# zju3dv/OnePose_Plus_Plus

Hardware: AMD Instinct MI355X
Metric: query images/sec (2D-3D match fwd) at 512x512 img x 5k pts (higher is better)
Workload: dtype f32 (operands as exact bf16 triples, f32 accumulate)

## Files before the change

onepose_plus_plus_amd/csrc/gemm_mfma.hip:

```cpp
#include <stdlib.h>

#include <mutex>
#include <type_traits>

#include <vector>

#include "opp_internal.h"

typedef float f32x16 __attribute__((ext_vector_type(16)));
typedef _Float16 f16x8 __attribute__((ext_vector_type(8)));
typedef __bf16 bf16x8 __attribute__((ext_vector_type(8)));
typedef __bf16 bf16x2 __attribute__((ext_vector_type(2)));
typedef float f32x2 __attribute__((ext_vector_type(2)));

namespace {

constexpr int lds_stride(int prec) { return prec == OPP_PREC_BF16X3 ? 52 : 36; }

__device__ __forceinline__ void opp_split4_b3(const float4 v, uint2& hi, uint2& mid, uint2& lo) {
  auto lvl = [](float a, float b, float& ra, float& rb) -> unsigned {
    const f32x2 t = {a, b};
    const unsigned p = __builtin_bit_cast(unsigned, __builtin_convertvector(t, bf16x2));
    ra = a - __uint_as_float(p << 16);
    rb = b - __uint_as_float(p & 0xffff0000u);
// ... 9 lines not shown
}
__device__ __forceinline__ void opp_store_split4(void* base, size_t row_bytes_off, int col, const float4 v) {
  uint2 hi, mid, lo;
  opp_split4_b3(v, hi, mid, lo);
  char* p = static_cast<char*>(base) + row_bytes_off + (col >> 3) * 48 + (col & 7) * 2;
  *reinterpret_cast<uint2*>(p) = hi;
  *reinterpret_cast<uint2*>(p + 16) = mid;
  *reinterpret_cast<uint2*>(p + 32) = lo;
}

template <int BM, int BN, int WAVES_M, int WAVES_N, bool CONV, int ABL, int DEPTH, int PREC, bool ASP>
__device__ __forceinline__ void opp_gemm_body(const OppGemm& g) {
  constexpr bool H2 = PREC == OPP_PREC_FP16X2;
  constexpr bool H3 = PREC == OPP_PREC_BF16X3;
  constexpr int kLdsStride = lds_stride(PREC);
  constexpr int NT = WAVES_M * WAVES_N * 64;
  constexpr int TM = BM / WAVES_M / 32;
  constexpr int NT32 = BN / 32;
  constexpr int TN = (NT32 + WAVES_N - 1) / WAVES_N;
  constexpr bool kRagged = (NT32 % WAVES_N) != 0;
  static_assert(!ASP || (CONV && PREC == OPP_PREC_BF16X3 && (ABL == 0 || ABL >= 200)), "pre-split activations: bf16x3 convolutions only");
  constexpr int kAblMask = ABL >= 200 ? ABL - 200 : 0;
  constexpr bool kNoGload = ABL == 91 || (kAblMask & 1), kNoLdsSt = ABL == 92 || (kAblMask & 2), kNoBar = ABL == 93 || (kAblMask & 4),
                 kNoFrag = ABL == 94 || (kAblMask & 8);
  constexpr int A_LD = ASP ? (BM * 12 + NT - 1) / NT : BM * 8 / NT;
  constexpr bool kAFrac = ASP && (BM * 12) % NT != 0;
  constexpr int kBRowsLoad = (H3 && BN == 224) ? 208 : BN;
  constexpr int B_LD = H3 ? (kBRowsLoad * 12 + NT - 1) / NT : BN * 8 / NT;
  constexpr bool kBFrac = H3 && (kBRowsLoad * 12) % NT != 0;
  constexpr bool kRing = H3 && kRagged && !CONV;
  constexpr bool kM16 = H3 && CONV;
  constexpr int NB16 = kM16 ? kBRowsLoad / 16 : 1;
  constexpr int NBW = kM16 ? (NB16 + WAVES_N - 1) / WAVES_N : 1;
  constexpr int MB = 2 * TM;
  static_assert(!kM16 || (kBRowsLoad % 16 == 0 && (!kRagged || WAVES_N == 2)), "16 x 16 tile shape");
  static_assert(BM % (WAVES_M * 32) == 0 && BN % 32 == 0, "tile shape");
  static_assert((BM * 8) % NT == 0 && (H3 ? (BN * 12) % NT == 0 || BN == 192 || BN == 224 : (BN * 8) % NT == 0), "load split");
  static_assert(!ASP || !((H3 && ((BN + 31) / 32 % WAVES_N) != 0)), "pre-split activations are not built for the ring tile");

  unsigned long long ts0 = 0, ts1 = 0, ts2 = 0;
  if (ABL == 9 || ABL > 90) ts0 = __builtin_readcyclecounter();
  extern __shared__ __attribute__((aligned(16))) float smem[];
  float* As = smem;
  float* Bs = smem + 2 * BM * kLdsStride;

  const int tid = threadIdx.x;
  const int lane = tid & 63;
  const int wave = tid >> 6;
  const int wm = __builtin_amdgcn_readfirstlane((H3 && kRagged) ? wave % WAVES_M : wave / WAVES_N);
  const int wn = __builtin_amdgcn_readfirstlane((H3 && kRagged) ? wave / WAVES_M : wave % WAVES_N);
  bool tile_ok[TN];
#pragma unroll
  for (int j = 0; j < TN; ++j) tile_ok[j] = kRagged ? (wn * TN + j < NT32) : true;
  const int half = lane >> 5;
  const int l31 = lane & 31;

  const int tiles_n = (g.n_store + BN - 1) / BN;
  int tile_lin = blockIdx.x;
  if (g.xcd_swizzle & 1) {
    const int nb = gridDim.x, q = nb >> 3, r = nb & 7;
    const int xcd = blockIdx.x & 7, idx = blockIdx.x >> 3;
    tile_lin = (xcd < r ? xcd * (q + 1) : r * (q + 1) + (xcd - r) * q) + idx;
  }
  const int tile_m = tile_lin / tiles_n;
  const int tile_n = tile_lin - tile_m * tiles_n;
  const int m0 = tile_m * BM;
  const int n0 = tile_n * BN;

// ... 9 lines not shown
#pragma unroll
  for (int i = 0; i < A_LD; ++i) {
    const int au = tid + i * NT;
    const int arow = ASP ? au / 12 : lrow + i * (NT / 8);
    const int apiece = ASP ? au - arow * 12 : 0;
    if constexpr (ASP) a_lds[i] = piece_off(arow, apiece);
    const int r = m0 + arow;
    if (CONV) {
      const int ox = r % g.Wout;
      const int t = r / g.Wout;
      const int oy = t % g.Hout;
      const int b = t / g.Hout;
      const int iy0 = oy * g.stride - g.pad;
      const int ix0 = ox * g.stride - g.pad;
      if constexpr (ASP) a_base0[i] = (unsigned)(((b * g.Hin + iy0) * g.Win + ix0) * g.Cin) * 6u + (unsigned)apiece * 16u;
      else a_base0[i] = (unsigned)(((b * g.Hin + iy0) * g.Win + ix0) * g.Cin + kq * 4) * 4u;
      a_base1[i] = 0;
      unsigned m = 0;
#pragma unroll
      for (int ky = 0; ky < 3; ++ky)
#pragma unroll
        for (int kx = 0; kx < 3; ++kx) {
          const bool ok = ky < g.ksize && kx < g.ksize && (unsigned)(iy0 + ky) < (unsigned)g.Hin &&
                          (unsigned)(ix0 + kx) < (unsigned)g.Win;
          m |= (ok ? 1u : 0u) << (ky * g.ksize + kx);
        }
      a_mask[i] = (r < g.M && (!kAFrac || au < BM * 12)) ? ~m : 0xffffffffu;
    } else {
      a_base0[i] = r < g.M ? (unsigned)(r * g.lda0 + kq * 4) * 4u : kOob;
      a_base1[i] = r < g.M ? (unsigned)(r * g.lda1 + kq * 4) * 4u : kOob;
      a_mask[i] = 0;
    }
  }
  constexpr bool kRingB = H3 && (NT32 % WAVES_N) != 0;
  unsigned b_base[kRingB ? 1 : B_LD];
  int b_lds[kRingB ? 1 : B_LD];
  auto ring_b = [&](int i, unsigned& base, int& lds) {
    int t = tid;
    asm volatile("" : "+v"(t));
    const int u = t + i * NT;
    const int row = u / 12, c = u - row * 12;
    const int n = n0 + row;
    base = (n < g.N && u < kBRowsLoad * 12) ? (unsigned)(n * g.ldw + c * 4) * 4u : kOob;
    lds = row * kLdsStride + c * 4;
  };
#pragma unroll
  for (int i = 0; i < (kRingB ? 0 : B_LD); ++i) {
    if (H3) {
      const int u = tid + i * NT;
      const int row = u / 12, c = u - row * 12;
      const int n = n0 + row;
      if constexpr (kBFrac) b_base[i] = (n < g.N && u < kBRowsLoad * 12) ? (unsigned)(n * g.ldw + c * 4) * 4u : kOob;
      else b_base[i] = n < g.N ? (unsigned)(n * g.ldw + c * 4) * 4u : kOob;
      b_lds[i] = piece_off(row, c);
    } else {
      const int n = n0 + lrow + i * (NT / 8);
      b_base[i] = n < g.N ? (unsigned)(n * g.ldw + kq * 4) * 4u : kOob;
      b_lds[i] = (lrow + i * (NT / 8)) * kLdsStride + kq * 4;
    }
  }

  typedef unsigned int u32x4 __attribute__((ext_vector_type(4)));
  auto bload = [](const __amdgpu_buffer_rsrc_t r, unsigned off) -> float4 {
    const u32x4 v = __builtin_amdgcn_raw_buffer_load_b128(r, (int)off, 0, 0);
    return make_float4(__uint_as_float(v.x), __uint_as_float(v.y), __uint_as_float(v.z), __uint_as_float(v.w));
  };

// ... 471 lines not shown
    mfma_ring(0, 2, 5, 2 * TM * TNW, tnw_c, pre);
    __builtin_amdgcn_sched_barrier(0);
    read_frags_n(B0, 4, fa[2], fb[2], tnw_c);
    __builtin_amdgcn_sched_barrier(0);
    mfma_ring(0, 5, 6, 5 * TM * TNW, tnw_c, pre);
#pragma unroll
    for (int i = kSlotsR0 / kStrideR0; i < A_LD; ++i) load_item(i, ga[P], gb[0]);
    __builtin_amdgcn_sched_barrier(0);
    mfma_ring(1, 0, 3, 0, tnw_c, [&](int n) {
      if (n % kStrideR1 == 0 && n / kStrideR1 < kItems) {
        store_item(n / kStrideR1, B1, ga[PN], gb[0]);
        __builtin_amdgcn_sched_barrier(0);
      }
    });
#pragma unroll
    for (int i = kSlotsR1 / kStrideR1; i < kItems; ++i) store_item(i, B1, ga[PN], gb[0]);
    __builtin_amdgcn_sched_barrier(0);
    __syncthreads();
    read_frags_n(B1, 0, fa[0], fb[0], tnw_c);
    read_frags_n(B1, 2, fa[3], fb[3], tnw_c);
    __builtin_amdgcn_sched_barrier(0);
    mfma_ring(1, 3, 5, 0, tnw_c, pre_b);
    __builtin_amdgcn_sched_barrier(0);
    read_frags_n(B1, 1, fa[2], fb[2], tnw_c);
    __builtin_amdgcn_sched_barrier(0);
    mfma_ring(1, 5, 6, 2 * TM * TNW, tnw_c, pre_b);
#pragma unroll
    for (int i = kSlotsR1 / kStrideRB; i < B_LD; ++i) load_item(A_LD + i, ga[P], gb[0]);
    __builtin_amdgcn_sched_barrier(0);
  };


  typedef float f32x4 __attribute__((ext_vector_type(4)));
  constexpr int NBH0 = (NBW + 1) / 2;
  f32x4 acc4[kM16 ? MB : 1][kM16 ? NBW : 1];
  float4 fa4[3][kM16 ? MB : 1], fb4[3][kM16 ? NBW : 1];
  if constexpr (kM16) {
#pragma unroll
    for (int i = 0; i < MB; ++i)
#pragma unroll
      for (int j = 0; j < NBW; ++j) acc4[i][j] = f32x4{0.f, 0.f, 0.f, 0.f};
  }
  const int f16off = (lane & 15) * kLdsStride + (((lane >> 4) ^ kswz(lane & 15)) * 3) * 4;
  const int a_frag16 = wm * TM * 32 * kLdsStride + f16off;
  const int b_frag16 = wn * NBW * 16 * kLdsStride + f16off;
  auto read_a16 = [&](int buf, auto h_c) {
    constexpr int H = decltype(h_c)::value;
    const float* as = As + buf * BM * kLdsStride + a_frag16;
#pragma unroll
    for (int i = H * TM; i < H * TM + TM; ++i)
#pragma unroll
      for (int p = 0; p < 3; ++p) fa4[p][i] = *reinterpret_cast<const float4*>(as + i * 16 * kLdsStride + p * 4);
  };
  auto read_b16 = [&](int buf, auto v_c, auto nbw_c) {
    constexpr int V = decltype(v_c)::value, NBL = decltype(nbw_c)::value;
    constexpr int j0 = V ? NBH0 : 0, j1 = V ? NBL : (NBH0 < NBL ? NBH0 : NBL);
    const float* bs = Bs + buf * BN * kLdsStride + b_frag16;
#pragma unroll
    for (int j = j0; j < j1; ++j)
#pragma unroll
      for (int p = 0; p < 3; ++p) fb4[p][j] = *reinterpret_cast<const float4*>(bs + j * 16 * kLdsStride + p * 4);
  };
  auto quad16 = [&](auto h_c, auto v_c, auto nbw_c, auto&& between) {
    constexpr int H = decltype(h_c)::value, V = decltype(v_c)::value, NBL = decltype(nbw_c)::value;
    constexpr int j0 = V ? NBH0 : 0, j1 = V ? NBL : (NBH0 < NBL ? NBH0 : NBL);
    constexpr int PA[6] = {2, 0, 1, 1, 0, 0};
    constexpr int PB[6] = {0, 2, 1, 0, 1, 0};
    int n = 0;
#pragma unroll
    for (int pr = 0; pr < 6; ++pr)
#pragma unroll
      for (int i = H * TM; i < H * TM + TM; ++i)
#pragma unroll
        for (int j = j0; j < j1; ++j) {
          acc4[i][j] = __builtin_amdgcn_mfma_f32_16x16x32_bf16(as_b8(fa4[PA[pr]][i]), as_b8(fb4[PB[pr]][j]), acc4[i][j], 0, 0, 0);
          between(n);
          ++n;
        }
  };
  auto chunk_m16 = [&](auto set, int lb, auto nbw_c) {
    constexpr int P = decltype(set)::value;
    constexpr int NBL = decltype(nbw_c)::value;
    constexpr int O = P & 1;
    constexpr int kSl0 = 6 * TM * (O ? NBL - NBH0 : (NBH0 < NBL ? NBH0 : NBL));
    constexpr int kSl1 = 6 * TM * (O ? (NBH0 < NBL ? NBH0 : NBL) : NBL - NBH0);
    constexpr int kSt0 = kSl0 / kItems > 0 ? kSl0 / kItems : 1;
    constexpr int kSt1 = kSl1 / kItems > 0 ? kSl1 / kItems : 1;
    using I0 = std::integral_constant<int, 0>;
    using I1 = std::integral_constant<int, 1>;
    const int B0 = lb, B1 = lb ^ 1;
    advance();
    if (!kNoFrag) {
      if constexpr (O == 0) read_b16(B0, I1{}, nbw_c);
      else read_b16(B0, I0{}, nbw_c);
      read_a16(B0, I1{});
    }
    __builtin_amdgcn_sched_barrier(0);
    auto hand = [&](int n) {
      if (n % kSt0 == 0 && n / kSt0 < kItems) {
        if (!kNoLdsSt) store_item(n / kSt0, B1, ga[0], gb[0]);
        __builtin_amdgcn_sched_barrier(0);
      }
    };
    auto pre = [&](int n) {
      if (n % kSt1 == 0 && n / kSt1 < kItems) {
        if (!kNoGload) load_item(n / kSt1, ga[0], gb[0]);
        __builtin_amdgcn_sched_barrier(0);
      }
    };
    if constexpr (O == 0) quad16(I0{}, I0{}, nbw_c, hand);
    else quad16(I0{}, I1{}, nbw_c, hand);
#pragma unroll
    for (int i = kSl0 / kSt0; i < kItems; ++i)
      if (!kNoLdsSt) store_item(i, B1, ga[0], gb[0]);
    __builtin_amdgcn_sched_barrier(0);
    if constexpr (O == 0) quad16(I0{}, I1{}, nbw_c, pre);
    else quad16(I0{}, I0{}, nbw_c, pre);
#pragma unroll
    for (int i = kSl1 / kSt1; i < kItems; ++i)
      if (!kNoGload) load_item(i, ga[0], gb[0]);
    __builtin_amdgcn_sched_barrier(0);
    if (!kNoBar) __syncthreads();
    if (!kNoFrag) read_a16(B1, I0{});
    __builtin_amdgcn_sched_barrier(0);
    if constexpr (O == 0) quad16(I1{}, I1{}, nbw_c, nothing);
    else quad16(I1{}, I0{}, nbw_c, nothing);
    __builtin_amdgcn_sched_barrier(0);
    if (!kNoFrag) {
      if constexpr (O == 0) read_b16(B1, I1{}, nbw_c);
      else read_b16(B1, I0{}, nbw_c);
    }
    __builtin_amdgcn_sched_barrier(0);
    if constexpr (O == 0) quad16(I1{}, I0{}, nbw_c, nothing);
    else quad16(I1{}, I1{}, nbw_c, nothing);
    __builtin_amdgcn_sched_barrier(0);
  };
  if constexpr (kM16) {
    if (!kNoFrag) {
      read_a16(0, std::integral_constant<int, 0>{});
      read_b16(0, std::integral_constant<int, 0>{}, std::integral_constant<int, NBW>{});
    }
  }

  if (ABL == 9 || ABL > 90) ts1 = __builtin_readcyclecounter();
  if (NT == 512 && (g.xcd_swizzle & 2) && __builtin_amdgcn_readfirstlane(tid) >= 256) __builtin_amdgcn_s_setprio(1);
  if constexpr (kRing) {
    constexpr int kFull = TN, kShort = NT32 - (WAVES_N - 1) * TN;
    static_assert(DEPTH == 2 && kShort >= 1 && kShort <= TN, "ring tile");
    if (wn != WAVES_N - 1) {
      for (int c = 0; c < nk; c += 2) {
        chunk_ring(std::integral_constant<int, 0>{}, c & 1, std::integral_constant<int, kFull>{});
        chunk_ring(std::integral_constant<int, 1>{}, (c + 1) & 1, std::integral_constant<int, kFull>{});
      }
    } else {
      for (int c = 0; c < nk; c += 2) {
        chunk_ring(std::integral_constant<int, 0>{}, c & 1, std::integral_constant<int, kShort>{});
        chunk_ring(std::integral_constant<int, 1>{}, (c + 1) & 1, std::integral_constant<int, kShort>{});
      }
    }
  }
  if constexpr (kM16) {
    static_assert(DEPTH == 2, "16 x 16 loop: the two quadrant orders alternate over a chunk pair");
    constexpr int kShort16 = NB16 - (WAVES_N - 1) * NBW;
    if (!kRagged || wn != WAVES_N - 1) {
      for (int c = 0; c < nk; c += 2) {
        chunk_m16(std::integral_constant<int, 0>{}, c & 1, std::integral_constant<int, NBW>{});
        chunk_m16(std::integral_constant<int, 1>{}, (c + 1) & 1, std::integral_constant<int, NBW>{});
      }
    } else {
      for (int c = 0; c < nk; c += 2) {
        chunk_m16(std::integral_constant<int, 0>{}, c & 1, std::integral_constant<int, kShort16>{});
        chunk_m16(std::integral_constant<int, 1>{}, (c + 1) & 1, std::integral_constant<int, kShort16>{});
      }
    }
  }
  for (int c = 0; c < ((kRing || kM16) ? 0 : nk); c += DEPTH) {
    if constexpr (kRing || kM16) {
    } else if constexpr (H3) {
      chunk_h3(std::integral_constant<int, 0>{}, c & 1);
      if (DEPTH > 1) chunk_h3(std::integral_constant<int, 1 % DEPTH>{}, (c + 1) & 1);
      if (DEPTH > 2) chunk_h3(std::integral_constant<int, 2 % DEPTH>{}, (c + 2) & 1);
      if (DEPTH > 3) chunk_h3(std::integral_constant<int, 3 % DEPTH>{}, (c + 3) & 1);
    } else if constexpr (H2) {
      chunk_h2(std::integral_constant<int, 0>{}, c & 1);
      if (DEPTH > 1) chunk_h2(std::integral_constant<int, 1 % DEPTH>{}, (c + 1) & 1);
      if (DEPTH > 2) chunk_h2(std::integral_constant<int, 2 % DEPTH>{}, (c + 2) & 1);
      if (DEPTH > 3) chunk_h2(std::integral_constant<int, 3 % DEPTH>{}, (c + 3) & 1);
    } else {
      chunk(std::integral_constant<int, 0>{}, c & 1);
      if (DEPTH > 1) chunk(std::integral_constant<int, 1 % DEPTH>{}, (c + 1) & 1);
      if (DEPTH > 2) chunk(std::integral_constant<int, 2 % DEPTH>{}, (c + 2) & 1);
      if (DEPTH > 3) chunk(std::integral_constant<int, 3 % DEPTH>{}, (c + 3) & 1);
    }
  }
  if (ABL == 9 || ABL > 90) ts2 = __builtin_readcyclecounter();
  if (ABL == 5) {
#pragma unroll
    for (int i = 0; i < A_LD; ++i) asm volatile("" ::"v"(da[i].x), "v"(da[i].w));
#pragma unroll
    for (int i = 0; i < B_LD; ++i) asm volatile("" ::"v"(db[i].x), "v"(db[i].w));
  }

  constexpr int kJPmax = TN < 4 ? TN : 4;
  constexpr int kOperandFloats = 2 * (BM + BN) * kLdsStride;
  constexpr int JP = (BM * (WAVES_N * kJPmax * 32 + 4) <= kOperandFloats) ? kJPmax
                     : (BM * (WAVES_N * 2 * 32 + 4) <= kOperandFloats && kJPmax >= 2) ? 2 : 1;
  constexpr int NPASS = kM16 ? 1 : (TN + JP - 1) / JP;
  constexpr int WP = kM16 ? BN : WAVES_N * JP * 32;
  constexpr int CS = WP + 4;
  static_assert((size_t)BM * CS * 4 <= (size_t)2 * (BM + BN) * kLdsStride * 4, "C tile must fit the operand LDS");
  float* Cs = smem;
  const bool scale_on = (g.out_mul != 1.f) || (g.out_div != 1.f);
  const bool vec_ok = g.vec_epilogue != 0;
  const float h2_inv = (H2 && g.h2_inv != nullptr) ? *g.h2_inv : 1.f;
  if constexpr (kM16) {
    if (scale_on) {
#pragma unroll
      for (int i = 0; i < MB; ++i)
#pragma unroll
        for (int j = 0; j < NBW; ++j)
#pragma unroll
          for (int r = 0; r < 4; ++r) acc4[i][j][r] = (acc4[i][j][r] * g.out_mul) / g.out_div;
    }
  } else if (H2 || scale_on) {
#pragma unroll
    for (int i = 0; i < TM; ++i)
#pragma unroll
      for (int j = 0; j < TN; ++j)
#pragma unroll
        for (int r = 0; r < 16; ++r) {
          const float cv0 = H2 ? acc[i][j][r] * h2_inv : acc[i][j][r];
          acc[i][j][r] = scale_on ? (cv0 * g.out_mul) / g.out_div : cv0;
        }
  }
  if (!kM16 && g.col_mask != nullptr) {
#pragma unroll
    for (int j = 0; j < TN; ++j) {
      const int col = n0 + wn * TN * 32 + j * 32 + l31;
      const float add = (col < g.n_store && g.col_mask[col] == 0.f) ? -1e9f : 0.f;
#pragma unroll
      for (int i = 0; i < TM; ++i)
#pragma unroll
        for (int r = 0; r < 16; ++r) acc[i][j][r] += add;
    }
  }
  if constexpr (H2) {
    if (g.nonfinite != nullptr) {
      bool bad = false;
#pragma unroll
      for (int i = 0; i < TM; ++i)
#pragma unroll
        for (int j = 0; j < TN; ++j)
#pragma unroll
          for (int r = 0; r < 16; ++r) bad |= !(fabsf(acc[i][j][r]) <= 3.4028235e38f);
      if (__builtin_amdgcn_ballot_w64(bad) != 0ull && lane == 0) atomicOr(g.nonfinite, 1);
    }
  }
#pragma unroll
  for (int ps = 0; ps < NPASS; ++ps) {
    __syncthreads();
    if constexpr (kM16) {
#pragma unroll
      for (int i = 0; i < MB; ++i)
#pragma unroll
        for (int j = 0; j < NBW; ++j)
#pragma unroll
          for (int r = 0; r < 4; ++r)
            Cs[(wm * TM * 32 + i * 16 + (lane >> 4) * 4 + r) * CS + wn * NBW * 16 + j * 16 + (lane & 15)] = acc4[i][j][r];
    } else
#pragma unroll
    for (int i = 0; i < TM; ++i)
#pragma unroll
      for (int jj = 0; jj < JP; ++jj) {
        const int j = ps * JP + jj;
        if (j < TN && tile_ok[j]) {
#pragma unroll
          for (int r = 0; r < 16; ++r) {
            const int lr = wm * TM * 32 + i * 32 + (r & 3) + 8 * (r >> 2) + 4 * half;
            Cs[lr * CS + wn * JP * 32 + jj * 32 + l31] = acc[i][j][r];
          }
        }
      }
    __syncthreads();
    if constexpr (!kM16 && NPASS == 1 && !kRagged && (NT % BM) == 0 && kOperandFloats - BM * CS >= 2 * (NT / BM) * BM + 2 * WAVES_M * WP) {
      if (g.stat_rowmax != nullptr) {
        constexpr int kParts = NT / BM;
        constexpr int kQ = WP / 4 / kParts;
        float* sc_r = Cs + BM * CS;
        float* sc_c = sc_r + 2 * kParts * BM;
        const int ncols = min(WP, g.n_store - n0);
        const int nrows = min(BM, g.M - m0);
        {
          const int lr = tid % BM, part = tid / BM;
          const float* rowp = Cs + lr * CS + part * kQ * 4;
          float mx = -INFINITY;
#pragma unroll 4
          for (int q = 0; q < kQ; ++q) {
            const float4 v = *reinterpret_cast<const float4*>(rowp + q * 4);
            const int c = (part * kQ + q) * 4;
            mx = fmaxf(mx, c + 0 < ncols ? v.x : -INFINITY);
            mx = fmaxf(mx, c + 1 < ncols ? v.y : -INFINITY);
            mx = fmaxf(mx, c + 2 < ncols ? v.z : -INFINITY);
            mx = fmaxf(mx, c + 3 < ncols ? v.w : -INFINITY);
          }
// ... 299 lines not shown
    }
    if (out != nullptr) out[i] = make_float4(v[0], v[1], v[2], v[3]);
  }
}

template <typename K>
void set_lds_once(K k, size_t lds, OppLdsOnce& once) {
  opp_lds_opt_in(reinterpret_cast<const void*>(k), lds, once);
}

template <int BM, int BN, int WAVES_M, int WAVES_N, int DEPTH, int PREC>
int launch_prec(const OppGemm& g, hipStream_t stream, size_t extra_lds) {
  constexpr int NT = WAVES_M * WAVES_N * 64;
  constexpr bool kNarrowB3 = BM == 128 && (BN == 192 || BN == 224) && NT == 512 && PREC == OPP_PREC_BF16X3;
  constexpr bool ok = (PREC == OPP_PREC_FP32 && BN != 192 && BN != 224) ||
                      (DEPTH == 2 && (NT == 512 || (BM == 64 && BN == 64) || (PREC == OPP_PREC_FP16X2 && BM == 128 && BN == 128)) &&
                       (BN == 128 || BN == 64 || BN == 256 || kNarrowB3) &&
                       (PREC != OPP_PREC_BF16X3 || (BN * 12) % NT == 0 || kNarrowB3) && (PREC != OPP_PREC_BF16X3 || BM * BN / NT <= 64 || kNarrowB3));
  if constexpr (ok) {
    const size_t lds = (size_t)2 * (BM + BN) * lds_stride(PREC) * sizeof(float) + extra_lds;
    const int tiles = opp_cdiv(g.M, BM) * opp_cdiv(g.n_store, BN);
    constexpr bool kAspBuilt = PREC == OPP_PREC_BF16X3 && DEPTH == 2 && !kNarrowB3 && (NT == 512 || (BM == 64 && BN == 64));
    if (g.conv && g.a_split) {
      if constexpr (kAspBuilt) {
        auto k = opp_gemm_asp_kernel<BM, BN, WAVES_M, WAVES_N, 0, DEPTH, PREC>;
        static OppLdsOnce attr_done;
        set_lds_once(k, lds, attr_done);
        hipLaunchKernelGGL(k, dim3(tiles, g.k_splits > 1 ? g.k_splits : 1), dim3(NT), lds, stream, g);
      } else {
        opp_set_error("gemm: tile %dx%d is not built for pre-split activations", BM, BN);
        return OPP_ERR_UNSUPPORTED;
      }
    } else if (g.conv) {
      if constexpr (PREC == OPP_PREC_BF16X3 && BN == 224) {
        opp_set_error("gemm: bf16x3 convolutions have no 224-column tile (config 27 runs them on 128 x 256)");
        return OPP_ERR_UNSUPPORTED;
      } else {
        auto k = opp_gemm_kernel<BM, BN, WAVES_M, WAVES_N, true, 0, DEPTH, PREC>;
        static OppLdsOnce attr_done;
        set_lds_once(k, lds, attr_done);
        hipLaunchKernelGGL(k, dim3(tiles, g.k_splits > 1 ? g.k_splits : 1), dim3(NT), lds, stream, g);
      }
    } else {
      auto k = opp_gemm_kernel<BM, BN, WAVES_M, WAVES_N, false, 0, DEPTH, PREC>;
      static OppLdsOnce attr_done;
      set_lds_once(k, lds, attr_done);
      hipLaunchKernelGGL(k, dim3(tiles, g.k_splits > 1 ? g.k_splits : 1), dim3(NT), lds, stream, g);
    }
    OPP_CHECK_LAUNCH("opp_gemm_kernel");
    return OPP_OK;
  } else {
    opp_set_error("gemm: tile %dx%d on %d waves is not built for operand precision %d", BM, BN, WAVES_M * WAVES_N, PREC);
    return OPP_ERR_UNSUPPORTED;
  }
}

template <int BM, int BN, int WAVES_M, int WAVES_N, int DEPTH = 2>
int launch_cfg(const OppGemm& g, hipStream_t stream) {
#ifdef OPP_TUNING
  static const size_t extra_lds = getenv("OPP_EXTRA_LDS") ? (size_t)atoi(getenv("OPP_EXTRA_LDS")) : 0;
#else
  constexpr size_t extra_lds = 0;
#endif
  switch (g.prec) {
    case OPP_PREC_FP32: return launch_prec<BM, BN, WAVES_M, WAVES_N, DEPTH, OPP_PREC_FP32>(g, stream, extra_lds);
#ifdef OPP_TUNING
    case OPP_PREC_FP16X2: return launch_prec<BM, BN, WAVES_M, WAVES_N, DEPTH, OPP_PREC_FP16X2>(g, stream, extra_lds);
#else
    case OPP_PREC_FP16X2: opp_set_error("gemm: fp16x2 operands are built into the tuning library only"); return OPP_ERR_UNSUPPORTED;
#endif
    case OPP_PREC_BF16X3: return launch_prec<BM, BN, WAVES_M, WAVES_N, DEPTH, OPP_PREC_BF16X3>(g, stream, extra_lds);
    default: opp_set_error("gemm: unknown operand precision %d", g.prec); return OPP_ERR_INVALID;
  }
}

#ifdef OPP_TUNING
unsigned long long* g_dbg_ts = nullptr;

template <int BM, int BN, int WM, int WN, int PREC, int ABL = 9, bool ASP = false>
int launch_timed(const OppGemm& g_in, hipStream_t stream) {
// ... 99 lines not shown
    long long best = -1;
    static const int on224_env = getenv("OPP_TILE_224") ? atoi(getenv("OPP_TILE_224")) : 1;
#ifdef OPP_TUNING
    static const int only_env = getenv("OPP_B3_ONLY_CFG") ? atoi(getenv("OPP_B3_ONLY_CFG")) : -1;
    static const int skip_env = getenv("OPP_B3_SKIP_BIG") ? atoi(getenv("OPP_B3_SKIP_BIG")) : 0;
#endif
    for (const Cand& c : cands) {
#ifdef OPP_TUNING
      if (only_env >= 0 && c.cfg != only_env && !(c.cfg == 2 && only_env != 2 && (long long)opp_cdiv(g.M, 64) * opp_cdiv(g.n_store, 64) <= 256)) continue;
      if (skip_env && (c.cfg == 20 || c.cfg == 22)) continue;
#endif
      if (c.bn == 256 && g.n_store <= 128) continue;
      if (c.bn == 192 && (!g.conv || g.n_store % 192 != 0)) continue;
      if (c.bn == 224 && g.a_split) continue;
      if (c.bn == 224 && (g.n_store != 224 || g.n_real <= 0 || g.n_real > 208 || on224_env == 0 ||
                          (on224_env != 2 && (g.tile_policy == OPP_TILES_THROUGHPUT || opp_cdiv(g.M, 128) < 256)))) continue;
      const long long tiles = (long long)opp_cdiv(g.M, c.bm) * opp_cdiv(g.n_store, c.bn);
      const long long slots = cus * c.wpc, full = tiles / slots, rem = tiles % slots;
      long long est = full * (nk * c.chunk * c.wpc + c.fixed);
      if (rem > 0) est += nk * c.chunk * ((rem + cus - 1) / cus) + c.fixed;
      if (g.tile_policy == OPP_TILES_THROUGHPUT) {
        if (tiles < 64 && c.cfg != 2) continue;
        est = tiles * (nk * c.chunk + c.fixed / c.wpc);
      }
      if (best < 0 || est < best) {
        best = est;
        cfg = c.cfg;
      }
    }
  }
  return cfg;
}

int opp_gemm_launch_cfg(const OppGemm& g_in, int cfg, hipStream_t stream) {
  OppGemm g = g_in;
  auto al16p = [](const void* p) { return (reinterpret_cast<uintptr_t>(p) & 15) == 0; };
  {
    auto al16 = [](const void* p) { return (reinterpret_cast<uintptr_t>(p) & 15) == 0; };
    bool v = g.n_store % 4 == 0 && (g.C == nullptr || (g.ldc % 4 == 0 && al16(g.C))) && (!g.bias || al16(g.bias)) && g.qk_cols % 4 == 0;
    if (g.res_mode != OPP_RES_NONE) v = v && g.ldr % 4 == 0 && al16(g.R);
    g.vec_epilogue = v ? 1 : 0;
  }
#ifdef OPP_TUNING
  static const int xcd_env = getenv("OPP_XCD_SWIZZLE") ? atoi(getenv("OPP_XCD_SWIZZLE")) : 1;
  g.xcd_swizzle = xcd_env;
#else
  g.xcd_swizzle = 1;
#endif
  {
    static const int prio_env = getenv("OPP_WAVE_PRIO") ? atoi(getenv("OPP_WAVE_PRIO")) : 0;
    if (prio_env) g.xcd_swizzle |= 2;
  }
  OPP_CHECK_ARG(g.M > 0 && g.N > 0 && g.K > 0 && g.K % 32 == 0, "gemm: bad M/N/K (%d,%d,%d)", g.M, g.N, g.K);
  OPP_CHECK_ARG(g.n_store >= g.N && (g.C || g.C3) && g.W && g.A0, "gemm: bad output/operands");
  OPP_CHECK_ARG((size_t)g.M * (size_t)g.ldc < (1ull << 31), "gemm: output too large for 32-bit indexing");
  if (g.C3 != nullptr || g.a_split) {
    OPP_CHECK_ARG(g.conv && g.prec == OPP_PREC_BF16X3, "gemm: pre-split activations are a bf16x3 convolution feature");
    OPP_CHECK_ARG(g.C3 == nullptr || (g.vec_epilogue && g.n_store % 8 == 0 && g.ld3 >= g.n_store * 6 && g.ld3 % 16 == 0 && al16p(g.C3) && !g.ln_gamma && !g.stat_rowmax &&
                                      g.k_splits <= 1), "gemm: split output needs the 16-byte epilogue, whole 8-channel groups and a plain launch");
    OPP_CHECK_ARG(!g.a_split || (g.tail_grp == 0 && al16p(g.A0)), "gemm: pre-split input needs Cin %% 32 == 0 real channels");
    OPP_CHECK_ARG(g.C != nullptr || g.C3 != nullptr, "gemm: no output");
  }
  g.w_bytes = (unsigned)((size_t)g.N * g.ldw * 4);
  OPP_CHECK_ARG((size_t)g.N * g.ldw * 4 < (1ull << 31), "gemm: weight operand too large for buffer addressing");
  OPP_CHECK_ARG(g.prec != OPP_PREC_BF16X3 || g.ldw * 2 >= g.K * 3, "gemm: bf16x3 weights need a row stride of 1.5 K floats");
  if (g.conv) {
// ... 42 lines not shown
      OPP_TRY(opp_gemm_launch_cfg(gs, 25, stream));
      const size_t n4 = (size_t)g.M * g.ldc / 4;
      const int blocks = (int)((n4 + 255) / 256 < 2048 ? (n4 + 255) / 256 : 2048);
      OppProfScope prof_epi(OPP_PROF_SPLITK_EPILOGUE, stream, (double)(kSplits + 1 + (g.res_mode == OPP_RES_DIRECT ? 1 : 0)) * (double)g.M * g.ldc * 4.0);
      hipLaunchKernelGGL(splitk_epilogue_kernel, dim3(blocks), dim3(256), 0, stream, reinterpret_cast<const float4*>(g.splitk_ws), kSplits, n4, n4, g.ldc / 4,
                         reinterpret_cast<const float4*>(g.bias), g.res_mode == OPP_RES_DIRECT ? reinterpret_cast<const float4*>(g.R) : nullptr, g.act,
                         reinterpret_cast<float4*>(g.C), g.C3, g.ld3);
      OPP_CHECK_LAUNCH("splitk_epilogue_kernel");
      return OPP_OK;
    }
  }
  const bool auto_cfg = cfg < 0;
  if (cfg < 0) cfg = choose_tile(g);
  OPP_CHECK_ARG(g.stat_rowmax == nullptr || (g.prec == OPP_PREC_BF16X3 ? (cfg == 25 || cfg == 20) : cfg == 0),
                "gemm: fused softmax statistics need the 128x128 tile (config 0; bf16x3: config 25, or 20 = 256x128)");
  if (g.ln_gamma != nullptr) {
    if (auto_cfg || (cfg != 30 && cfg != 26)) cfg = g.n_store == 256 ? 30 : 26;
    auto al = [](const void* p) { return (reinterpret_cast<uintptr_t>(p) & 15) == 0; };
    OPP_CHECK_ARG(g.ln_beta && ((cfg == 30 && g.n_store == 256) || (cfg == 26 && g.n_store == 128)) && g.N == g.n_store && !g.bias &&
                      g.act == OPP_ACT_NONE && g.res_mode == OPP_RES_NONE && g.ldc % 4 == 0 && al(g.C) && al(g.ln_gamma) &&
                      al(g.ln_beta) && (!g.ln_res || (al(g.ln_res) && g.ln_ldres % 4 == 0)),
                  "gemm: fused LayerNorm needs a 256- or 128-column output, no bias/activation/residual mode, aligned operands");
  }
  OppProfScope prof_scope(g.conv && g.k_splits > 1 ? (int)OPP_PROF_CONV_SPLITK : opp_prof_gemm_symbol(cfg, g.conv ? 1 : (g.stat_rowmax ? 2 : 0)), stream,
                          g.alg_flops > 0.0 ? g.alg_flops : 2.0 * (double)g.M * (double)g.N * (double)g.K);
  int rc;
  switch (cfg) {
    case 0: rc = launch_cfg<128, 128, 2, 2>(g, stream); break;
    case 1: rc = launch_cfg<64, 128, 2, 2>(g, stream); break;
    case 2: rc = launch_cfg<64, 64, 2, 2>(g, stream); break;
    case 10: rc = launch_cfg<128, 128, 2, 2, 3>(g, stream); break;
    case 11: rc = launch_cfg<128, 128, 2, 2, 4>(g, stream); break;
    case 20: rc = launch_cfg<256, 128, 4, 2>(g, stream); break;
    case 22: rc = launch_cfg<128, 256, 2, 4>(g, stream); break;
    case 24: rc = launch_cfg<128, 192, 4, 2>(g, stream); break;
    case 25: rc = launch_cfg<128, 128, 4, 2>(g, stream); break;
    case 27:
      if (g.prec != OPP_PREC_BF16X3 || g.n_store > 224 || (g.n_real > 208 && g.n_real != g.n_store)) {
        opp_set_error("gemm: tile config 27 (128 x 224) is a bf16x3 tile for outputs of <= 208 real and <= 224 stored columns");
        rc = OPP_ERR_UNSUPPORTED;
      } else if (g.conv && g.prec == OPP_PREC_BF16X3) {
        rc = launch_cfg<128, 256, 2, 4>(g, stream);
      } else {
        rc = launch_cfg<128, 224, 4, 2>(g, stream);
      }
      break;
    case 26: rc = launch_cfg<64, 128, 2, 4>(g, stream); break;
    case 30: rc = launch_cfg<64, 256, 2, 4>(g, stream); break;
    default:
#ifdef OPP_TUNING
      rc = launch_tuning_cfg(g, cfg, stream);
#else
      opp_set_error("gemm: unknown tile config %d", cfg);
      rc = OPP_ERR_INVALID;
#endif
      break;
  }
  return rc;
}

extern "C" int opp_debug_timestamps(void* buf) {
#ifdef OPP_TUNING
  g_dbg_ts = static_cast<unsigned long long*>(buf);
  opp_gemm_ss_debug_timestamps(buf, getenv("OPP_SS_TS_MODE") ? atoi(getenv("OPP_SS_TS_MODE")) : 0);
  return OPP_OK;
#else
  (void)buf;
  opp_set_error("opp_debug_timestamps: library built without -DOPP_TUNING");
  return OPP_ERR_UNSUPPORTED;
#endif
}

int opp_gemm_launch(const OppGemm& g, hipStream_t stream) { return opp_gemm_launch_cfg(g, -1, stream); }

int opp_gemm_choose_tile(const OppGemm& g) {
// ... 5 lines not shown
```

Measured before the change: 575.5.

## Add two-role 128x224 bf16x3 conv tile for outputs of at most 208 columns

Adds a 128x224 tile for bf16x3 convolutions with at most 208 real output columns. Four waves each compute a 64x64 block over columns 0-127 and the other four each compute a 32x80 block over columns 128-207, so no MFMA work is spent on padding columns 208-255 as in the earlier 128x256 fallback. The 16x16 inner loop is refactored into a per-wave templated lambda that stages its accumulators into LDS itself, and padding columns are zero-filled. Configs 22 and 27 route eligible conv GEMMs to the new tile. The uneven wave roles may unbalance the work per wave and change register pressure.

```diff
diff --git a/onepose_plus_plus_amd/csrc/gemm_mfma.hip b/onepose_plus_plus_amd/csrc/gemm_mfma.hip
--- a/onepose_plus_plus_amd/csrc/gemm_mfma.hip
+++ b/onepose_plus_plus_amd/csrc/gemm_mfma.hip
@@ -65,8 +65,8 @@
   constexpr bool kM16 = H3 && CONV;
   constexpr int NB16 = kM16 ? kBRowsLoad / 16 : 1;
   constexpr int NBW = kM16 ? (NB16 + WAVES_N - 1) / WAVES_N : 1;
-  constexpr int MB = 2 * TM;
-  static_assert(!kM16 || (kBRowsLoad % 16 == 0 && (!kRagged || WAVES_N == 2)), "16 x 16 tile shape");
+  constexpr bool kRoles = kM16 && BM == 128 && BN == 224 && WAVES_M == 2 && WAVES_N == 4;
+  static_assert(!kM16 || (kBRowsLoad % 16 == 0 && (!kRagged || WAVES_N == 2 || kRoles)), "16 x 16 tile shape");
   static_assert(BM % (WAVES_M * 32) == 0 && BN % 32 == 0, "tile shape");
   static_assert((BM * 8) % NT == 0 && (H3 ? (BN * 12) % NT == 0 || BN == 192 || BN == 224 : (BN * 8) % NT == 0), "load split");
   static_assert(!ASP || !((H3 && ((BN + 31) / 32 % WAVES_N) != 0)), "pre-split activations are not built for the ring tile");
@@ -142,7 +142,7 @@
       a_mask[i] = 0;
     }
   }
-  constexpr bool kRingB = H3 && (NT32 % WAVES_N) != 0;
+  constexpr bool kRingB = kRing;
   unsigned b_base[kRingB ? 1 : B_LD];
   int b_lds[kRingB ? 1 : B_LD];
   auto ring_b = [&](int i, unsigned& base, int& lds) {
@@ -680,118 +680,142 @@
 
 
   typedef float f32x4 __attribute__((ext_vector_type(4)));
-  constexpr int NBH0 = (NBW + 1) / 2;
-  f32x4 acc4[kM16 ? MB : 1][kM16 ? NBW : 1];
-  float4 fa4[3][kM16 ? MB : 1], fb4[3][kM16 ? NBW : 1];
-  if constexpr (kM16) {
-#pragma unroll
-    for (int i = 0; i < MB; ++i)
-#pragma unroll
-      for (int j = 0; j < NBW; ++j) acc4[i][j] = f32x4{0.f, 0.f, 0.f, 0.f};
-  }
   const int f16off = (lane & 15) * kLdsStride + (((lane >> 4) ^ kswz(lane & 15)) * 3) * 4;
-  const int a_frag16 = wm * TM * 32 * kLdsStride + f16off;
-  const int b_frag16 = wn * NBW * 16 * kLdsStride + f16off;
-  auto read_a16 = [&](int buf, auto h_c) {
-    constexpr int H = decltype(h_c)::value;
-    const float* as = As + buf * BM * kLdsStride + a_frag16;
-#pragma unroll
-    for (int i = H * TM; i < H * TM + TM; ++i)
-#pragma unroll
-      for (int p = 0; p < 3; ++p) fa4[p][i] = *reinterpret_cast<const float4*>(as + i * 16 * kLdsStride + p * 4);
-  };
-  auto read_b16 = [&](int buf, auto v_c, auto nbw_c) {
-    constexpr int V = decltype(v_c)::value, NBL = decltype(nbw_c)::value;
-    constexpr int j0 = V ? NBH0 : 0, j1 = V ? NBL : (NBH0 < NBL ? NBH0 : NBL);
-    const float* bs = Bs + buf * BN * kLdsStride + b_frag16;
-#pragma unroll
-    for (int j = j0; j < j1; ++j)
-#pragma unroll
-      for (int p = 0; p < 3; ++p) fb4[p][j] = *reinterpret_cast<const float4*>(bs + j * 16 * kLdsStride + p * 4);
-  };
-  auto quad16 = [&](auto h_c, auto v_c, auto nbw_c, auto&& between) {
-    constexpr int H = decltype(h_c)::value, V = decltype(v_c)::value, NBL = decltype(nbw_c)::value;
-    constexpr int j0 = V ? NBH0 : 0, j1 = V ? NBL : (NBH0 < NBL ? NBH0 : NBL);
-    constexpr int PA[6] = {2, 0, 1, 1, 0, 0};
-    constexpr int PB[6] = {0, 2, 1, 0, 1, 0};
-    int n = 0;
-#pragma unroll
-    for (int pr = 0; pr < 6; ++pr)
-#pragma unroll
-      for (int i = H * TM; i < H * TM + TM; ++i)
-#pragma unroll
-        for (int j = j0; j < j1; ++j) {
-          acc4[i][j] = __builtin_amdgcn_mfma_f32_16x16x32_bf16(as_b8(fa4[PA[pr]][i]), as_b8(fb4[PB[pr]][j]), acc4[i][j], 0, 0, 0);
-          between(n);
-          ++n;
-        }
-  };
-  auto chunk_m16 = [&](auto set, int lb, auto nbw_c) {
-    constexpr int P = decltype(set)::value;
-    constexpr int NBL = decltype(nbw_c)::value;
-    constexpr int O = P & 1;
-    constexpr int kSl0 = 6 * TM * (O ? NBL - NBH0 : (NBH0 < NBL ? NBH0 : NBL));
-    constexpr int kSl1 = 6 * TM * (O ? (NBH0 < NBL ? NBH0 : NBL) : NBL - NBH0);
-    constexpr int kSt0 = kSl0 / kItems > 0 ? kSl0 / kItems : 1;
-    constexpr int kSt1 = kSl1 / kItems > 0 ? kSl1 / kItems : 1;
-    using I0 = std::integral_constant<int, 0>;
-    using I1 = std::integral_constant<int, 1>;
-    const int B0 = lb, B1 = lb ^ 1;
-    advance();
-    if (!kNoFrag) {
-      if constexpr (O == 0) read_b16(B0, I1{}, nbw_c);
-      else read_b16(B0, I0{}, nbw_c);
-      read_a16(B0, I1{});
-    }
-    __builtin_amdgcn_sched_barrier(0);
-    auto hand = [&](int n) {
-      if (n % kSt0 == 0 && n / kSt0 < kItems) {
-        if (!kNoLdsSt) store_item(n / kSt0, B1, ga[0], gb[0]);
-        __builtin_amdgcn_sched_barrier(0);
-      }
+  auto loop_start = [&]() {
+    if (ABL == 9 || ABL > 90) ts1 = __builtin_readcyclecounter();
+    if (NT == 512 && (g.xcd_swizzle & 2) && __builtin_amdgcn_readfirstlane(tid) >= 256) __builtin_amdgcn_s_setprio(1);
+  };
+  auto m16_tile = [&](auto tm_c, auto nbw_c, auto nbl_c, int arow0, int bcol0) __attribute__((always_inline)) {
+    constexpr int TMW = decltype(tm_c)::value, NBWW = decltype(nbw_c)::value, NBLW = decltype(nbl_c)::value;
+    constexpr int MBW = 2 * TMW;
+    constexpr int NBH0 = (NBWW + 1) / 2;
+    f32x4 acc4[MBW][NBWW];
+    float4 fa4[3][MBW], fb4[3][NBWW];
+#pragma unroll
+    for (int i = 0; i < MBW; ++i)
+#pragma unroll
+      for (int j = 0; j < NBWW; ++j) acc4[i][j] = f32x4{0.f, 0.f, 0.f, 0.f};
+    const int a_frag16 = arow0 * kLdsStride + f16off;
+    const int b_frag16 = bcol0 * kLdsStride + f16off;
+    auto read_a16 = [&](int buf, auto h_c) {
+      constexpr int H = decltype(h_c)::value;
+      const float* as = As + buf * BM * kLdsStride + a_frag16;
+#pragma unroll
+      for (int i = H * TMW; i < H * TMW + TMW; ++i)
+#pragma unroll
+        for (int p = 0; p < 3; ++p) fa4[p][i] = *reinterpret_cast<const float4*>(as + i * 16 * kLdsStride + p * 4);
     };
-    auto pre = [&](int n) {
-      if (n % kSt1 == 0 && n / kSt1 < kItems) {
-        if (!kNoGload) load_item(n / kSt1, ga[0], gb[0]);
-        __builtin_amdgcn_sched_barrier(0);
-      }
+    auto read_b16 = [&](int buf, auto v_c) {
+      constexpr int V = decltype(v_c)::value;
+      constexpr int j0 = V ? NBH0 : 0, j1 = V ? NBLW : (NBH0 < NBLW ? NBH0 : NBLW);
+      const float* bs = Bs + buf * BN * kLdsStride + b_frag16;
+#pragma unroll
+      for (int j = j0; j < j1; ++j)
+#pragma unroll
+        for (int p = 0; p < 3; ++p) fb4[p][j] = *reinterpret_cast<const float4*>(bs + j * 16 * kLdsStride + p * 4);
     };
-    if constexpr (O == 0) quad16(I0{}, I0{}, nbw_c, hand);
-    else quad16(I0{}, I1{}, nbw_c, hand);
-#pragma unroll
-    for (int i = kSl0 / kSt0; i < kItems; ++i)
-      if (!kNoLdsSt) store_item(i, B1, ga[0], gb[0]);
-    __builtin_amdgcn_sched_barrier(0);
-    if constexpr (O == 0) quad16(I0{}, I1{}, nbw_c, pre);
-    else quad16(I0{}, I0{}, nbw_c, pre);
-#pragma unroll
-    for (int i = kSl1 / kSt1; i < kItems; ++i)
-      if (!kNoGload) load_item(i, ga[0], gb[0]);
-    __builtin_amdgcn_sched_barrier(0);
-    if (!kNoBar) __syncthreads();
-    if (!kNoFrag) read_a16(B1, I0{});
-    __builtin_amdgcn_sched_barrier(0);
-    if constexpr (O == 0) quad16(I1{}, I1{}, nbw_c, nothing);
-    else quad16(I1{}, I0{}, nbw_c, nothing);
-    __builtin_amdgcn_sched_barrier(0);
-    if (!kNoFrag) {
-      if constexpr (O == 0) read_b16(B1, I1{}, nbw_c);
-      else read_b16(B1, I0{}, nbw_c);
-    }
-    __builtin_amdgcn_sched_barrier(0);
-    if constexpr (O == 0) quad16(I1{}, I0{}, nbw_c, nothing);
-    else quad16(I1{}, I1{}, nbw_c, nothing);
-    __builtin_amdgcn_sched_barrier(0);
-  };
-  if constexpr (kM16) {
+    auto quad16 = [&](auto h_c, auto v_c, auto&& between) {
+      constexpr int H = decltype(h_c)::value, V = decltype(v_c)::value;
+      constexpr int j0 = V ? NBH0 : 0, j1 = V ? NBLW : (NBH0 < NBLW ? NBH0 : NBLW);
+      constexpr int PA[6] = {2, 0, 1, 1, 0, 0};
+      constexpr int PB[6] = {0, 2, 1, 0, 1, 0};
+      int n = 0;
+#pragma unroll
+      for (int pr = 0; pr < 6; ++pr)
+#pragma unroll
+        for (int i = H * TMW; i < H * TMW + TMW; ++i)
+#pragma unroll
+          for (int j = j0; j < j1; ++j) {
+            acc4[i][j] = __builtin_amdgcn_mfma_f32_16x16x32_bf16(as_b8(fa4[PA[pr]][i]), as_b8(fb4[PB[pr]][j]), acc4[i][j], 0, 0, 0);
+            between(n);
+            ++n;
+          }
+    };
+    auto chunk_m16 = [&](auto set, int lb) {
+      constexpr int P = decltype(set)::value;
+      constexpr int O = P & 1;
+      constexpr int kSl0 = 6 * TMW * (O ? NBLW - NBH0 : (NBH0 < NBLW ? NBH0 : NBLW));
+      constexpr int kSl1 = 6 * TMW * (O ? (NBH0 < NBLW ? NBH0 : NBLW) : NBLW - NBH0);
+      constexpr int kSt0 = kSl0 / kItems > 0 ? kSl0 / kItems : 1;
+      constexpr int kSt1 = kSl1 / kItems > 0 ? kSl1 / kItems : 1;
+      using I0 = std::integral_constant<int, 0>;
+      using I1 = std::integral_constant<int, 1>;
+      const int B0 = lb, B1 = lb ^ 1;
+      advance();
+      if (!kNoFrag) {
+        if constexpr (O == 0) read_b16(B0, I1{});
+        else read_b16(B0, I0{});
+        read_a16(B0, I1{});
+      }
+      __builtin_amdgcn_sched_barrier(0);
+      auto hand = [&](int n) {
+        if (n % kSt0 == 0 && n / kSt0 < kItems) {
+          if (!kNoLdsSt) store_item(n / kSt0, B1, ga[0], gb[0]);
+          __builtin_amdgcn_sched_barrier(0);
+        }
+      };
+      auto pre = [&](int n) {
+        if (n % kSt1 == 0 && n / kSt1 < kItems) {
+          if (!kNoGload) load_item(n / kSt1, ga[0], gb[0]);
+          __builtin_amdgcn_sched_barrier(0);
+        }
+      };
+      if constexpr (O == 0) quad16(I0{}, I0{}, hand);
+      else quad16(I0{}, I1{}, hand);
+#pragma unroll
+      for (int i = kSl0 / kSt0; i < kItems; ++i)
+        if (!kNoLdsSt) store_item(i, B1, ga[0], gb[0]);
+      __builtin_amdgcn_sched_barrier(0);
+      if constexpr (O == 0) quad16(I0{}, I1{}, pre);
+      else quad16(I0{}, I0{}, pre);
+#pragma unroll
+      for (int i = kSl1 / kSt1; i < kItems; ++i)
+        if (!kNoGload) load_item(i, ga[0], gb[0]);
+      __builtin_amdgcn_sched_barrier(0);
+      if (!kNoBar) __syncthreads();
+      if (!kNoFrag) read_a16(B1, I0{});
+      __builtin_amdgcn_sched_barrier(0);
+      if constexpr (O == 0) quad16(I1{}, I1{}, nothing);
+      else quad16(I1{}, I0{}, nothing);
+      __builtin_amdgcn_sched_barrier(0);
+      if (!kNoFrag) {
+        if constexpr (O == 0) read_b16(B1, I1{});
+        else read_b16(B1, I0{});
+      }
+      __builtin_amdgcn_sched_barrier(0);
+      if constexpr (O == 0) quad16(I1{}, I0{}, nothing);
+      else quad16(I1{}, I1{}, nothing);
+      __builtin_amdgcn_sched_barrier(0);
+    };
     if (!kNoFrag) {
       read_a16(0, std::integral_constant<int, 0>{});
-      read_b16(0, std::integral_constant<int, 0>{}, std::integral_constant<int, NBW>{});
-    }
-  }
-
-  if (ABL == 9 || ABL > 90) ts1 = __builtin_readcyclecounter();
-  if (NT == 512 && (g.xcd_swizzle & 2) && __builtin_amdgcn_readfirstlane(tid) >= 256) __builtin_amdgcn_s_setprio(1);
+      read_b16(0, std::integral_constant<int, 0>{});
+    }
+    loop_start();
+    for (int c = 0; c < nk; c += 2) {
+      chunk_m16(std::integral_constant<int, 0>{}, c & 1);
+      chunk_m16(std::integral_constant<int, 1>{}, (c + 1) & 1);
+    }
+    if (ABL == 9 || ABL > 90) ts2 = __builtin_readcyclecounter();
+    if (g.out_mul != 1.f || g.out_div != 1.f) {
+#pragma unroll
+      for (int i = 0; i < MBW; ++i)
+#pragma unroll
+        for (int j = 0; j < NBWW; ++j)
+#pragma unroll
+          for (int r = 0; r < 4; ++r) acc4[i][j][r] = (acc4[i][j][r] * g.out_mul) / g.out_div;
+    }
+    __syncthreads();
+#pragma unroll
+    for (int i = 0; i < MBW; ++i)
+#pragma unroll
+      for (int j = 0; j < NBWW; ++j)
+#pragma unroll
+        for (int r = 0; r < 4; ++r)
+          smem[(arow0 + i * 16 + (lane >> 4) * 4 + r) * (BN + 4) + bcol0 + j * 16 + (lane & 15)] = acc4[i][j][r];
+  };
+
+  if constexpr (!kM16) loop_start();
   if constexpr (kRing) {
     constexpr int kFull = TN, kShort = NT32 - (WAVES_N - 1) * TN;
     static_assert(DEPTH == 2 && kShort >= 1 && kShort <= TN, "ring tile");
@@ -809,17 +833,24 @@
   }
   if constexpr (kM16) {
     static_assert(DEPTH == 2, "16 x 16 loop: the two quadrant orders alternate over a chunk pair");
-    constexpr int kShort16 = NB16 - (WAVES_N - 1) * NBW;
-    if (!kRagged || wn != WAVES_N - 1) {
-      for (int c = 0; c < nk; c += 2) {
-        chunk_m16(std::integral_constant<int, 0>{}, c & 1, std::integral_constant<int, NBW>{});
-        chunk_m16(std::integral_constant<int, 1>{}, (c + 1) & 1, std::integral_constant<int, NBW>{});
-      }
+    using I1 = std::integral_constant<int, 1>;
+    using I2 = std::integral_constant<int, 2>;
+    using I4 = std::integral_constant<int, 4>;
+    using I5 = std::integral_constant<int, 5>;
+    if constexpr (kRoles) {
+      static_assert(TM == 2 && NB16 == 13, "two-role tile: 64 x 64 waves over columns 0 .. 127, 32 x 80 waves over 128 .. 207");
+      const int w = __builtin_amdgcn_readfirstlane(wave);
+      if (w < 4) m16_tile(I2{}, I4{}, I4{}, 64 * (w & 1), 64 * (w >> 1));
+      else m16_tile(I1{}, I5{}, I5{}, 32 * (w - 4), 128);
+      constexpr int kZq = (BN - NB16 * 16) / 4;
+      for (int u = tid; u < BM * kZq; u += NT)
+        *reinterpret_cast<float4*>(smem + (u / kZq) * (BN + 4) + NB16 * 16 + (u % kZq) * 4) = make_float4(0.f, 0.f, 0.f, 0.f);
     } else {
-      for (int c = 0; c < nk; c += 2) {
-        chunk_m16(std::integral_constant<int, 0>{}, c & 1, std::integral_constant<int, kShort16>{});
-        chunk_m16(std::integral_constant<int, 1>{}, (c + 1) & 1, std::integral_constant<int, kShort16>{});
-      }
+      constexpr int kShort16 = NB16 - (WAVES_N - 1) * NBW;
+      using IT = std::integral_constant<int, TM>;
+      using IW = std::integral_constant<int, NBW>;
+      if (!kRagged || wn != WAVES_N - 1) m16_tile(IT{}, IW{}, IW{}, wm * TM * 32, wn * NBW * 16);
+      else m16_tile(IT{}, IW{}, std::integral_constant<int, kShort16>{}, wm * TM * 32, wn * NBW * 16);
     }
   }
   for (int c = 0; c < ((kRing || kM16) ? 0 : nk); c += DEPTH) {
@@ -841,7 +872,7 @@
       if (DEPTH > 3) chunk(std::integral_constant<int, 3 % DEPTH>{}, (c + 3) & 1);
     }
   }
-  if (ABL == 9 || ABL > 90) ts2 = __builtin_readcyclecounter();
+  if (!kM16 && (ABL == 9 || ABL > 90)) ts2 = __builtin_readcyclecounter();
   if (ABL == 5) {
 #pragma unroll
     for (int i = 0; i < A_LD; ++i) asm volatile("" ::"v"(da[i].x), "v"(da[i].w));
@@ -857,20 +888,12 @@
   constexpr int WP = kM16 ? BN : WAVES_N * JP * 32;
   constexpr int CS = WP + 4;
   static_assert((size_t)BM * CS * 4 <= (size_t)2 * (BM + BN) * kLdsStride * 4, "C tile must fit the operand LDS");
+  static_assert(!kM16 || CS == BN + 4, "the 16 x 16 loop stages its accumulators with row stride BN + 4 (m16_tile)");
   float* Cs = smem;
   const bool scale_on = (g.out_mul != 1.f) || (g.out_div != 1.f);
   const bool vec_ok = g.vec_epilogue != 0;
   const float h2_inv = (H2 && g.h2_inv != nullptr) ? *g.h2_inv : 1.f;
-  if constexpr (kM16) {
-    if (scale_on) {
-#pragma unroll
-      for (int i = 0; i < MB; ++i)
-#pragma unroll
-        for (int j = 0; j < NBW; ++j)
-#pragma unroll
-          for (int r = 0; r < 4; ++r) acc4[i][j][r] = (acc4[i][j][r] * g.out_mul) / g.out_div;
-    }
-  } else if (H2 || scale_on) {
+  if (!kM16 && (H2 || scale_on)) {
 #pragma unroll
     for (int i = 0; i < TM; ++i)
 #pragma unroll
@@ -906,18 +929,9 @@
   }
 #pragma unroll
   for (int ps = 0; ps < NPASS; ++ps) {
-    __syncthreads();
-    if constexpr (kM16) {
-#pragma unroll
-      for (int i = 0; i < MB; ++i)
-#pragma unroll
-        for (int j = 0; j < NBW; ++j)
-#pragma unroll
-          for (int r = 0; r < 4; ++r)
-            Cs[(wm * TM * 32 + i * 16 + (lane >> 4) * 4 + r) * CS + wn * NBW * 16 + j * 16 + (lane & 15)] = acc4[i][j][r];
-    } else
-#pragma unroll
-    for (int i = 0; i < TM; ++i)
+    if constexpr (!kM16) __syncthreads();
+#pragma unroll
+    for (int i = 0; i < (kM16 ? 0 : TM); ++i)
 #pragma unroll
       for (int jj = 0; jj < JP; ++jj) {
         const int j = ps * JP + jj;
@@ -1283,8 +1297,8 @@
         return OPP_ERR_UNSUPPORTED;
       }
     } else if (g.conv) {
-      if constexpr (PREC == OPP_PREC_BF16X3 && BN == 224) {
-        opp_set_error("gemm: bf16x3 convolutions have no 224-column tile (config 27 runs them on 128 x 256)");
+      if constexpr (PREC == OPP_PREC_BF16X3 && BN == 224 && WAVES_N != 4) {
+        opp_set_error("gemm: the 128 x 224 ring tile is built for dense GEMMs only");
         return OPP_ERR_UNSUPPORTED;
       } else {
         auto k = opp_gemm_kernel<BM, BN, WAVES_M, WAVES_N, true, 0, DEPTH, PREC>;
@@ -1293,10 +1307,15 @@
         hipLaunchKernelGGL(k, dim3(tiles, g.k_splits > 1 ? g.k_splits : 1), dim3(NT), lds, stream, g);
       }
     } else {
-      auto k = opp_gemm_kernel<BM, BN, WAVES_M, WAVES_N, false, 0, DEPTH, PREC>;
-      static OppLdsOnce attr_done;
-      set_lds_once(k, lds, attr_done);
-      hipLaunchKernelGGL(k, dim3(tiles, g.k_splits > 1 ? g.k_splits : 1), dim3(NT), lds, stream, g);
+      if constexpr (BN == 224 && WAVES_N == 4) {
+        opp_set_error("gemm: the 128 x 224 two-role tile is built for bf16x3 convolutions only");
+        return OPP_ERR_UNSUPPORTED;
+      } else {
+        auto k = opp_gemm_kernel<BM, BN, WAVES_M, WAVES_N, false, 0, DEPTH, PREC>;
+        static OppLdsOnce attr_done;
+        set_lds_once(k, lds, attr_done);
+        hipLaunchKernelGGL(k, dim3(tiles, g.k_splits > 1 ? g.k_splits : 1), dim3(NT), lds, stream, g);
+      }
     }
     OPP_CHECK_LAUNCH("opp_gemm_kernel");
     return OPP_OK;
@@ -1462,6 +1481,10 @@
   return cfg;
 }
 
+static bool conv208(const OppGemm& g) {
+  return g.conv && g.prec == OPP_PREC_BF16X3 && !g.a_split && g.k_splits <= 1 && g.n_real > 0 && g.n_real <= 208 && g.n_store <= 224;
+}
+
 int opp_gemm_launch_cfg(const OppGemm& g_in, int cfg, hipStream_t stream) {
   OppGemm g = g_in;
   auto al16p = [](const void* p) { return (reinterpret_cast<uintptr_t>(p) & 15) == 0; };
@@ -1570,15 +1593,19 @@
     case 10: rc = launch_cfg<128, 128, 2, 2, 3>(g, stream); break;
     case 11: rc = launch_cfg<128, 128, 2, 2, 4>(g, stream); break;
     case 20: rc = launch_cfg<256, 128, 4, 2>(g, stream); break;
-    case 22: rc = launch_cfg<128, 256, 2, 4>(g, stream); break;
+    case 22:
+      rc = conv208(g) ? launch_cfg<128, 224, 2, 4>(g, stream) : launch_cfg<128, 256, 2, 4>(g, stream);
+      break;
     case 24: rc = launch_cfg<128, 192, 4, 2>(g, stream); break;
     case 25: rc = launch_cfg<128, 128, 4, 2>(g, stream); break;
     case 27:
       if (g.prec != OPP_PREC_BF16X3 || g.n_store > 224 || (g.n_real > 208 && g.n_real != g.n_store)) {
         opp_set_error("gemm: tile config 27 (128 x 224) is a bf16x3 tile for outputs of <= 208 real and <= 224 stored columns");
         rc = OPP_ERR_UNSUPPORTED;
-      } else if (g.conv && g.prec == OPP_PREC_BF16X3) {
+      } else if (g.conv && (g.a_split || g.k_splits > 1)) {
         rc = launch_cfg<128, 256, 2, 4>(g, stream);
+      } else if (g.conv) {
+        rc = launch_cfg<128, 224, 2, 4>(g, stream);
       } else {
         rc = launch_cfg<128, 224, 4, 2>(g, stream);
       }
```

Result: faster. 586.2, median of 6 (+1.9%).
